# kit-cel/gr-gfdm

Hardware: AMD Instinct MI355X
Metric: GFDM blocks/s, K=64 M=9 mod+demod (MF), batch 4096 per GPU (higher is better)
Workload: dtype f32; 1 GPU; BASELINE configs[1]: K=64 subcarriers, M=9 timeslots, RRC alpha=0.2, overlap=2, MF receiver, step = modulate + demodulate; 4096 QPSK blocks per step per GPU, ring of 36 buffer sets, independent steps pipelined over 3 HIP streams; block_size=576, batch_per_gpu=4096, streams=3

## Files before the change

gr-gfdm_amd/csrc/gfdm_jit.hip:

```cpp
#include "gfdm_rowvariants.h"

#include <hip/hiprtc.h>

#include <fcntl.h>
#include <pthread.h>
#include <sys/stat.h>
#include <unistd.h>

#include <cstdio>
#include <cstdlib>
#include <cstring>
#include <atomic>
#include <condition_variable>
#include <deque>
#include <map>
#include <memory>
#include <mutex>
#include <thread>
#include <string>
#include <tuple>
#include <vector>

namespace gfdm {
namespace {

struct Header { const char* name; const char* text; };
const Header kHeaders[] = {
#include "gfdm_jit_sources.inc"
};
constexpr int kNumHeaders = sizeof(kHeaders) / sizeof(kHeaders[0]);
#define GFDM_JIT_STR_I(x) #x
#define GFDM_JIT_STR(x) GFDM_JIT_STR_I(x)
const char* const kOptions[] = { "--offload-arch=gfx950", "-O3", "-std=c++17", "-fno-slp-vectorize",
                                 "-DGFDM_PACKED_TWT=" GFDM_JIT_STR(GFDM_PACKED_TWT), "-DGFDM_PACKED_ROOTS=" GFDM_JIT_STR(GFDM_PACKED_ROOTS) };
constexpr int kNumOptions = sizeof(kOptions) / sizeof(kOptions[0]);

std::vector<std::string> part_kernels(int K, int M, int L, int part)
{
    char buf[160];
    std::vector<std::string> v;
    const rowvar::PartVariants t = rowvar::part_variants(K, M, part);
    for (int i = 0; i < t.n; ++i) {
        const rowvar::Variant& k = t.v[i];
        if (part == JIT_PART_MOD) snprintf(buf, sizeof buf, "gfdm::jit::k_row_modulate<%d, %d, %d, %d>", K, M, L, k.tx);
        else if (part == JIT_PART_EST) snprintf(buf, sizeof buf, "gfdm::jit::k_row_estimate<%d, %d>", K, M);
        else if (part == JIT_PART_RX_BURST) snprintf(buf, sizeof buf, "gfdm::jit::k_row_receive_burst<%d, %d, %d, %d, %d>", K, M, L, k.mode, k.ick);
        else snprintf(buf, sizeof buf, "gfdm::jit::k_row_receive<%d, %d, %d, %d, %d, %d>", K, M, L, k.mode, k.eq, k.ick);
        v.push_back(buf);
    }
    return v;
}

uint64_t fnv1a(uint64_t h, const void* data, size_t n)
{
    const unsigned char* p = static_cast<const unsigned char*>(data);
    for (size_t i = 0; i < n; ++i) { h ^= p[i]; h *= 1099511628211ull; }
    return h;
}

uint64_t source_hash()
{
    static const uint64_t h = [] {
        uint64_t x = 1469598103934665603ull;
        for (int i = 0; i < kNumHeaders; ++i) x = fnv1a(x, kHeaders[i].text, strlen(kHeaders[i].text));
        for (int i = 0; i < kNumOptions; ++i) x = fnv1a(x, kOptions[i], strlen(kOptions[i]));
        int major = 0, minor = 0;
        (void)hiprtcVersion(&major, &minor);
        x = fnv1a(x, &major, sizeof major);
        return fnv1a(x, &minor, sizeof minor);
    }();
    return h;
}

std::string cache_dir()
{
    std::string d;
    if (const char* e = getenv("GFDM_HIP_CACHE_DIR")) d = e;
    else if (const char* x = getenv("XDG_CACHE_HOME")) d = std::string(x) + "/gfdm_hip";
    else if (const char* h = getenv("HOME")) d = std::string(h) + "/.cache/gfdm_hip";
    if (d.empty()) return d;
    struct stat st;
    if (lstat(d.c_str(), &st) != 0)
        for (size_t i = 1; i <= d.size(); ++i)
            if (i == d.size() || d[i] == '/') (void)mkdir(d.substr(0, i).c_str(), i == d.size() ? 0700 : 0755);
    if (lstat(d.c_str(), &st) != 0 || !S_ISDIR(st.st_mode) || st.st_uid != getuid() || (st.st_mode & (S_IWGRP | S_IWOTH))) return std::string();
    return d;
}
// ... 365 lines not shown
```

gr-gfdm_amd/csrc/gfdm_rowgeom.h:

```cpp
#pragma once
#ifndef __HIPCC_RTC__
#include <stddef.h>
#endif

#ifndef GFDM_ROW_WG
#define GFDM_ROW_WG 256
#endif

namespace gfdm {
namespace rowgeom {

constexpr bool pow2(int K) { return K > 0 && (K & (K - 1)) == 0; }
constexpr int ldiv(int K, int lim)
{
    int r = 1;
    for (int d = 2; d <= lim && d <= K; ++d)
        if (K % d == 0) r = d;
    return r;
}
constexpr bool plan2(int K, int lim) { return K / ldiv(K, lim) <= lim; }
constexpr bool plan3(int K, int lim) { return ldiv(K, lim) > 1 && ldiv(K / ldiv(K, lim), lim) > 1 && plan2(K / ldiv(K, lim), lim); }
constexpr int plan_lim(int K) { return ((K <= 256 && plan2(K, 16)) || plan3(K, 16)) ? 16 : 32; }
constexpr bool mixed(int K)
{
    return !pow2(K) && K >= 3 && K <= 1024 && ((K <= 256 && plan2(K, 16)) || (!plan3(K, 16) && plan2(K, 32)));
}
constexpr int mixed_r1(int K) { return ldiv(K, plan_lim(K)); }
constexpr int mixed_r0(int K) { return K / mixed_r1(K); }
constexpr bool mixed3(int K)
{
    return !pow2(K) && !mixed(K) && K >= 3 && K <= 1024 && (plan3(K, 16) || plan3(K, 32));
}
constexpr int mixed3_r2(int K) { return ldiv(K, plan_lim(K)); }
constexpr int mixed3_r1(int K) { return ldiv(K / mixed3_r2(K), plan_lim(K)); }
constexpr int mixed3_r0(int K) { return K / mixed3_r2(K) / mixed3_r1(K); }
constexpr bool supported(int K) { return (pow2(K) && K >= 4 && K <= 1024) || mixed(K) || mixed3(K); }

constexpr int wg(int K) { return K >= 128 ? K : pow2(K) ? GFDM_ROW_WG : (GFDM_ROW_WG / K) * K; }
constexpr bool wave_local(int K) { return K <= 64 && 64 % K == 0; }
constexpr int bpw(int K) { return wg(K) / K; }
constexpr int tile_stride(int K, int M) { return K * M + (bpw(K) > 1 ? 16 : 0); }
constexpr size_t lds_bytes(int K, int M) { return (size_t)bpw(K) * (size_t)tile_stride(K, M) * 8 + 64; }
constexpr bool ic_mfma(int K, int M) { return pow2(K) && K >= 16 && M >= 4 && M <= 16; }
constexpr bool ic_mfma_preferred(int K, int M) { return ic_mfma(K, M) && K >= 128; }
constexpr size_t ic_mfma_pad_bytes(int K) { return wave_local(K) ? 0 : (size_t)(K / 4) * 8; }
constexpr size_t ic_mfma_edge_bytes(int K) { return wave_local(K) ? 0 : (size_t)2 * (K / 64) * 2 * 2 * 4 * 8 + ic_mfma_pad_bytes(K); }
constexpr int est_stride(int K) { return K + 10; }
constexpr size_t est_bytes(int K) { return (size_t)bpw(K) * (size_t)est_stride(K) * 8; }

#ifndef GFDM_PACKED_TWT
#define GFDM_PACKED_TWT 1
#endif
#ifndef GFDM_PACKED_ROOTS
#define GFDM_PACKED_ROOTS 0
#endif
constexpr int wide_r0(int K) { return K == 256 ? 16 : K == 128 ? 8 : mixed(K) ? mixed_r0(K) : mixed3(K) ? mixed3_r0(K) : (K == 512 || K == 1024) ? 8 : 1; }
constexpr int wide_r1(int K) { return (K == 256 || K == 128) ? 16 : mixed(K) ? mixed_r1(K) : mixed3(K) ? mixed3_r1(K) : (K == 512 || K == 1024) ? 8 : 1; }
constexpr bool wide3(int K) { return K == 512 || K == 1024 || mixed3(K); }
constexpr bool wide(int K) { return K == 256 || K == 128 || mixed(K) || wide3(K); }
constexpr int root_count(int K)
{
    if (wide(K)) return (wide_r0(K) - 1) + (wide3(K) ? wide_r1(K) - 1 : 0);
    if (K == 64) return 3;
    int n = 0;
    for (int len = K; len >= 4; len /= 4)
        if (len / 4 > 1) n += 3;
    return n;
}
constexpr int root_index(int K, int lane, int i)
{
    if (wide(K)) {
        const int R0 = wide_r0(K), R1 = wide_r1(K);
        if (i < R0 - 1) return (lane % (K / R0)) * (i + 1) % K;
        return ((lane % (K / R1)) / R0) * R0 * (i - (R0 - 1) + 1) % K;
    }
    int str = 1;
    for (int s = 0; s < i / 3; ++s) str *= 4;
    return ((lane % (K / 4)) / str) * (i % 3 + 1) * str % K;
}
constexpr bool packed_twt(int K, int M)
{
    return GFDM_PACKED_TWT != 0 && M >= 3 && !(K == 128 && (M == 15 || M == 21)) && !(K == 4 && M == 16);
}
constexpr bool packed_roots(int K, int M)
{
    return GFDM_PACKED_ROOTS != 0 && root_count(K) >= 2 && !(K == 128 && M == 15) && !(K == 96 && M == 25);
}
constexpr size_t packed_elems(int n, int K) { return ((size_t)n * (size_t)K + 1) & ~(size_t)1; }
constexpr size_t packed_roots_offset(int K, int M) { return packed_elems(M, K); }

}
}
```

gr-gfdm_amd/csrc/gfdm_rowlane_impl.h:

```cpp
#pragma once
#include "gfdm_dft.h"
#include "gfdm_plan.h"
#include "gfdm_tx.h"
#include "gfdm_est.h"
#include "gfdm_burstfetch.h"
#include "gfdm_rowgeom.h"

#ifndef __HIPCC_RTC__
#include <cstdlib>
#endif

#ifdef __HIPCC_RTC__
#define GFDM_ROWLANE_NS jit
#else
#define GFDM_ROWLANE_NS
#endif

#ifndef GFDM_ROW_WG
#define GFDM_ROW_WG 256
#endif

namespace gfdm {
namespace GFDM_ROWLANE_NS {

using namespace dft;

#ifdef GFDM_STAMPS
__device__ unsigned long long* g_stamp_buf = nullptr;
#define GFDM_STAMP(slot)                                                                                         \
    do {                                                                                                         \
        asm volatile("s_waitcnt vmcnt(0) lgkmcnt(0)" ::: "memory");                                              \
        if (g_stamp_buf && (threadIdx.x & 63) == 0)                                                               \
            g_stamp_buf[((size_t)blockIdx.x * (blockDim.x / 64) + (threadIdx.x >> 6)) * 8 + (slot)] = __builtin_amdgcn_s_memrealtime(); \
    } while (0)
#else
#define GFDM_STAMP(slot) do { } while (0)
#endif

template <int K> struct RowShape {
    static_assert(rowgeom::supported(K), "row-lane family: K a power of two 4 .. 1024, or K <= 1024 a product of two or three factors <= 32 (gfdm_rowgeom.h)");
    static constexpr bool MIXED3 = rowgeom::mixed3(K);
    static constexpr bool MIXED = rowgeom::mixed(K);
    static constexpr int R0 = MIXED ? rowgeom::mixed_r0(K) : 1, R1 = MIXED ? rowgeom::mixed_r1(K) : 1;
    static constexpr int log2K = (K == 4) ? 2 : (K == 8) ? 3 : (K == 16) ? 4 : (K == 32) ? 5 : (K == 64) ? 6 : (K == 128) ? 7 : (K == 256) ? 8 : (K == 512) ? 9 : (K == 1024) ? 10 : 0;
    static constexpr int NP4 = log2K / 2;
    static constexpr bool HAS2 = (log2K & 1) != 0;
    static constexpr int WG = rowgeom::wg(K);
    static constexpr int BPW = rowgeom::bpw(K);
    static constexpr int RG = K / 4;
    static constexpr bool RADIX16 = (K == 256);
    static constexpr bool RADIX8X16 = (K == 128);
    static constexpr bool WIDE3 = (K == 512 || K == 1024) || MIXED3;
    static constexpr bool WIDE = RADIX16 || RADIX8X16 || MIXED || WIDE3;
    static constexpr int WIDE_R0 = (RADIX16 ? 16 : RADIX8X16 ? 8 : MIXED ? R0 : MIXED3 ? rowgeom::mixed3_r0(K) : WIDE3 ? 8 : 1);
    static constexpr int WIDE_R1 = (RADIX16 || RADIX8X16) ? 16 : MIXED ? R1 : MIXED3 ? rowgeom::mixed3_r1(K) : WIDE3 ? 8 : 1;
    static constexpr int WIDE_R2 = MIXED3 ? rowgeom::mixed3_r2(K) : WIDE3 ? K / 64 : 1;
    static constexpr bool LDS_REDUCE = MIXED || MIXED3;
};

template <int K>
__device__ __forceinline__ int wrap_k(int x)
{
    if constexpr (rowgeom::pow2(K)) return x & (K - 1); else return x % K;
}

constexpr int pow4(int s) { return 1 << (2 * s); }

template <int K>
__device__ __forceinline__ void block_sync()
{
    if constexpr (rowgeom::wave_local(K)) {
        __builtin_amdgcn_fence(__ATOMIC_ACQ_REL, "wavefront");
        __builtin_amdgcn_wave_barrier();
    } else {
        __syncthreads();
    }
}

template <int K, int M> struct RowTile {
    static constexpr int N = K * M;
    static constexpr int TS = rowgeom::tile_stride(K, M);
};

template <int K, int M> constexpr size_t row_lds_bytes() { return rowgeom::lds_bytes(K, M); }

template <int K> struct EstTile {
    static constexpr int FS = rowgeom::est_stride(K);
    static constexpr size_t bytes = rowgeom::est_bytes(K);
};

template <int K> struct FftLayout {
    static __device__ __forceinline__ int slot(int row)
    {
        if constexpr (RowShape<K>::RADIX8X16) {
            const int a = (row >> 5) & 3, c = row & 7;
            return (row & ~7) | ((c + 2 * a) & 7);
        } else if constexpr (RowShape<K>::RADIX16) {
            return (row & ~15) | ((row + (row >> 4)) & 15);
        } else if constexpr (K >= 64 && rowgeom::pow2(K) && !RowShape<K>::WIDE3) {
            const int b = (row >> 4) & 3, c = (row >> 2) & 3, d = row & 3;
            return (row & ~63) | (16 * b + 4 * ((c + b) & 3) + ((d + b) & 3));
        } else {
            return row;
        }
    }
};

template <int K> struct FftTwiddles {
    cf w[RowShape<K>::WIDE ? 1 : RowShape<K>::NP4][3];
    cf w16[RowShape<K>::WIDE_R0 > 1 ? RowShape<K>::WIDE_R0 - 1 : 1];
    cf wmid[RowShape<K>::WIDE3 ? RowShape<K>::WIDE_R1 - 1 : 1];
};

template <int K, int N, class F>
__device__ __forceinline__ void load_lane_packed(const cf* __restrict__ tab, int q, F&& put)
{
    static_for<0, N / 2>([&](auto ji) {
        constexpr int j = decltype(ji)::value;
        const v4f_io w = *reinterpret_cast<const v4f_io*>(tab + 2 * (j * K + q));
        put(std::integral_constant<int, 2 * j>{}, mk(w.x, w.y));
        put(std::integral_constant<int, 2 * j + 1>{}, mk(w.z, w.w));
    });
    if constexpr (N % 2 != 0) put(std::integral_constant<int, N - 1>{}, tab[(N / 2) * 2 * K + q]);
}

template <int K, int M>
__device__ __forceinline__ void load_row_twiddles(cf (&tw)[M], const cf* __restrict__ twT, int q)
{
    if constexpr (rowgeom::packed_twt(K, M)) load_lane_packed<K, M - 1>(twT, q, [&](auto ii, cf w) { tw[decltype(ii)::value + 1] = w; });
    else static_for<1, M>([&](auto mi) { constexpr int m = decltype(mi)::value; tw[m] = twT[m * K + q]; });
}
// ... 293 lines not shown

#ifndef GFDM_WIDE_MOD_IN
#define GFDM_WIDE_MOD_IN 1
#endif
#ifndef GFDM_WIDE_RX_OUT
#define GFDM_WIDE_RX_OUT 0
#endif
#ifndef GFDM_WIDE_RX_IN
#define GFDM_WIDE_RX_IN 0
#endif
#ifndef GFDM_WIDE_MOD_OUT
#define GFDM_WIDE_MOD_OUT 0
#endif
constexpr bool kWideModIn = GFDM_WIDE_MOD_IN != 0, kWideRxOut = GFDM_WIDE_RX_OUT != 0, kWideRxIn = GFDM_WIDE_RX_IN != 0, kWideModOut = GFDM_WIDE_MOD_OUT != 0;

__device__ __forceinline__ float dpp_pair_swap(float x)
{
    return __builtin_bit_cast(float, __builtin_amdgcn_update_dpp(0, __builtin_bit_cast(int, x), 0xB1, 0xF, 0xF, true));
}
__device__ __forceinline__ cf dpp_pair_swap(cf x) { return mk(dpp_pair_swap(x.x), dpp_pair_swap(x.y)); }

template <int M>
__device__ __forceinline__ void wide_block_to_tile(cf* X, const cf* __restrict__ src, int l)
{
    v4f_io w[M / 2 > 0 ? M / 2 : 1];
    cf tail = mk(0.f, 0.f);
    static_for<0, M / 2>([&](auto ii) { constexpr int i = decltype(ii)::value; w[i] = ld_stream2(src + 2 * (l + 64 * i)); });
    if constexpr (M % 2) tail = ld_stream(src + 64 * (M - 1) + l);
    static_for<0, M / 2>([&](auto ii) { constexpr int i = decltype(ii)::value; reinterpret_cast<v4f_io*>(X)[l + 64 * i] = w[i]; });
    if constexpr (M % 2) X[64 * (M - 1) + l] = tail;
}
template <int M>
__device__ __forceinline__ void wide_tile_to_block(cf* __restrict__ dst, int64_t base, const cf* X, int l)
{
    static_for<0, M / 2>([&](auto ii) { constexpr int i = decltype(ii)::value; st_stream2(dst, base + 2 * (l + 64 * i), reinterpret_cast<const v4f_io*>(X)[l + 64 * i]); });
    if constexpr (M % 2) st_stream(dst, base + 64 * (M - 1) + l, X[64 * (M - 1) + l]);
}

template <int M>
__device__ __forceinline__ void wide_load_rows(cf (&v)[M], const cf* __restrict__ src, int l)
{
    const bool odd = (l & 1) != 0;
    const cf* p = src + 64 * (l & 1) + (l & ~1);
    v4f_io w[M / 2 > 0 ? M / 2 : 1];
    static_for<0, M / 2>([&](auto ii) { constexpr int i = decltype(ii)::value; w[i] = ld_stream2(p + 128 * i); });
    if constexpr (M % 2) v[M - 1] = ld_stream(src + 64 * (M - 1) + l);
    static_for<0, M / 2>([&](auto ii) {
        constexpr int i = decltype(ii)::value;
        const cf a = mk(w[i].x, w[i].y), b = mk(w[i].z, w[i].w);
        const cf got = dpp_pair_swap(odd ? a : b);
        v[2 * i] = odd ? got : a;
        v[2 * i + 1] = odd ? b : got;
    });
}
template <int M>
__device__ __forceinline__ void wide_store_rows(cf* __restrict__ dst, int64_t base, const cf (&v)[M], int l)
{
    const bool odd = (l & 1) != 0;
    const int64_t at = base + 64 * (l & 1) + (l & ~1);
    static_for<0, M / 2>([&](auto ii) {
        constexpr int i = decltype(ii)::value;
        const cf got = dpp_pair_swap(odd ? v[2 * i] : v[2 * i + 1]);
        const cf a = odd ? got : v[2 * i], b = odd ? v[2 * i + 1] : got;
        st_stream2(dst, at + 128 * i, v4f_io{ a.x, a.y, b.x, b.y });
    });
    if constexpr (M % 2) st_stream(dst, base + 64 * (M - 1) + l, v[M - 1]);
}

template <bool TREAL>
__device__ __forceinline__ cf tap_fma(cf t, cf x, cf c)
{
    if constexpr (TREAL) return mk(fmaf(t.x, x.x, c.x), fmaf(t.x, x.y, c.y)); else return cfma(t, x, c);
}

__device__ __forceinline__ cf decide_point(cf x, const IcParams& ic)
{
    if (ic.decision == 1) {
        const float s = 0.70710678118654752f;
        return mk(x.x > 0.f ? s : -s, x.y > 0.f ? s : -s);
    }
    int idx = 0;
    if (ic.decision == 2) {
        idx = (x.x > 0.f);
    } else {
        float best = __builtin_huge_valf();
        for (int i = 0; i < ic.npoints; ++i) {
            const cf pt = ic.points[i];
            const float dr = x.x - pt.x, di = x.y - pt.y, d = dr * dr + di * di;
            if (d < best) { best = d; idx = i; }
        }
    }
    return ic.points[idx];
}



#ifndef GFDM_IC_REG_TRANSPOSE
#define GFDM_IC_REG_TRANSPOSE 0
#endif
constexpr bool kIcRegTranspose = GFDM_IC_REG_TRANSPOSE != 0;

typedef _Float16 ic_h8 __attribute__((ext_vector_type(8)));
typedef float ic_f4 __attribute__((ext_vector_type(4)));

template <int K, int M> struct IcMfma {
    static constexpr int KW = K < 64 ? K : 64;
// ... 128 lines not shown
                    cur[g4][c] = __builtin_amdgcn_mfma_f32_16x16x32_f16(afrag, nb, c0[g4][c], 0, 0, 0);
                    cur[g4][c] = __builtin_amdgcn_mfma_f32_16x16x32_f16(afrag2, nb, cur[g4][c], 0, 0, 0);
                });
            });
        }
        static_for<0, 4>([&](auto gi) {
            constexpr int g4 = decltype(gi)::value;
            cf* row = reinterpret_cast<cf*>(blk0) + grp_block(g4) * TS + pa(wbase + G * cn + (g4 % G), 4 * cr);
            static_for<0, 4>([&](auto ii) {
                constexpr int i = decltype(ii)::value;
                if (12 + i < M || 4 * cr + i < M) row[i] = mk(cur[g4][0][i], cur[g4][1][i]);
            });
        });
        block_sync<K>();
    }
};

#ifndef GFDM_IC_WAVES_PER_SIMD
#define GFDM_IC_WAVES_PER_SIMD 2
#endif
template <int K, int M, int EQ> constexpr int ic_mfma_waves_per_simd()
{
    constexpr size_t lds = ((EQ == EQ_PREAMBLE || EQ == EQ_BURST) ? rowgeom::lds_bytes(K, M + 2) + rowgeom::est_bytes(K) : rowgeom::lds_bytes(K, M)) + rowgeom::ic_mfma_edge_bytes(K);
    constexpr size_t per_cu = (160 * 1024) / ((lds + 511) / 512 * 512) * (size_t)(rowgeom::wg(K) / 64);
    return per_cu >= 4 * (size_t)GFDM_IC_WAVES_PER_SIMD ? GFDM_IC_WAVES_PER_SIMD : 2;
}
#ifndef GFDM_VALU_IC_WAVES_PER_SIMD
#define GFDM_VALU_IC_WAVES_PER_SIMD 1
#endif
#define GFDM_ROW_RECEIVE_BOUNDS(EQ_) __launch_bounds__(RowShape<K>::WG, ((MODE == RX_IC && ICK == ICK_MFMA) ? ic_mfma_waves_per_simd<K, M, EQ_>() : (MODE == RX_IC && K <= 64) ? GFDM_VALU_IC_WAVES_PER_SIMD : 1))
template <int K, int M, int L, int MODE, int EQT, int ICK>
__global__ GFDM_ROW_RECEIVE_BOUNDS(EQT) void k_row_receive(DevicePlan p, IcParams ic, EstPlan est, const cf* __restrict__ twT,
                                                                cf* __restrict__ out, const cf* __restrict__ in,
                                                                const cf* __restrict__ f_eq, int64_t nblocks)
{
    const BurstIo bio{};
#include "gfdm_rowlane_receive_body.h"
}

template <int K, int M, int L, int MODE, int ICK>
__global__ GFDM_ROW_RECEIVE_BOUNDS(EQ_BURST) void k_row_receive_burst(DevicePlan p, IcParams ic, EstPlan est, const cf* __restrict__ twT,
                                                                cf* __restrict__ out, const cf* __restrict__ in,
                                                                const cf* __restrict__ f_eq, int64_t nblocks, BurstIo bio)
{
    constexpr int EQT = EQ_BURST;
#include "gfdm_rowlane_receive_body.h"
}
#undef GFDM_ROW_RECEIVE_BOUNDS

template <int K, int M, int L, int TXMODE>
__global__ __launch_bounds__(RowShape<K>::WG) void k_row_modulate(DevicePlan p, TxParams tx, const cf* __restrict__ twT,
                                                                 cf* __restrict__ out, const cf* __restrict__ in, int64_t nblocks)
{
    using S = RowShape<K>;
    using T = RowTile<K, M>;
    constexpr int N = K * M;
    constexpr int PART = (M * L / 2 < M) ? (M * L / 2) : M;
    extern __shared__ __attribute__((aligned(16))) unsigned char smem[];
    const int g = threadIdx.x / K, q = threadIdx.x - g * K;
    const int64_t blk = (int64_t)blockIdx.x * S::BPW + g;
    const bool valid = blk < nblocks;
    const int64_t base = (valid ? blk : 0) * N;
    cf* X = reinterpret_cast<cf*>(smem) + g * T::TS;

    FftTwiddles<K> twd;
    load_fft_twiddles<K, rowgeom::packed_roots(K, M)>(twd, q, p.wK);
    constexpr bool PRE_TW = (M <= 16), PRE_TAPS = (L * M <= 24);
    cf twv[M], tapv[PRE_TAPS ? L * M : 1];
    if constexpr (PRE_TW) load_row_twiddles<K, M>(twv, twT, q);
    if constexpr (PRE_TAPS) static_for<0, L * M>([&](auto ii) { constexpr int i = decltype(ii)::value; tapv[i] = p.taps[i]; });
    auto tap = [&](auto ii) { constexpr int i = decltype(ii)::value; if constexpr (PRE_TAPS) return tapv[i]; else return p.taps[i]; };
    constexpr bool WIDE_IN = (K == 64 && TXMODE == 0 && kWideModIn), WIDE_OUT = (K == 64 && TXMODE == 0 && kWideModOut);
    const bool treal = (K == 64) ? (p.taps_real & PLAN_TAPS_REAL) != 0 : p.taps_real != 0;
    const bool wide = (K == 64) && (p.taps_real & PLAN_WIDE_IO) != 0;
    (void)wide;
    cf v[M];
    if constexpr (TXMODE == 0) {
        bool copied = false;
        if constexpr (WIDE_IN) {
            if (wide) { wide_block_to_tile<M>(X, in + base, q); copied = true; }
        }
        if (!copied) static_for<0, M>([&](auto ii) { constexpr int i = decltype(ii)::value; X[q + K * i] = ld_stream(in + base + q + K * i); });
        block_sync<K>();
        static_for<0, M>([&](auto mi) { constexpr int m = decltype(mi)::value; v[m] = X[q * M + m]; });
    } else {
        const cf* sym = in + (valid ? blk : 0) * (int64_t)tx.nin;
        static_for<0, M>([&](auto mi) { constexpr int m = decltype(mi)::value; v[m] = tx_symbol(tx, sym, M, q, m); });
    }
    dft_inplace<M, false>(v);
    constexpr float invN = 1.0f / (float)N;
    if constexpr (!(K == 64 && L == 2)) {
        static_for<0, M>([&](auto mi) { constexpr int m = decltype(mi)::value; X[q * M + m] = v[m]; });
        block_sync<K>();
    }
    auto filter = [&](auto real_tag) {
        constexpr bool TREAL = decltype(real_tag)::value;
        if constexpr (K == 64 && L == 2) {
            static_for<0, M>([&](auto mi) {
                constexpr int m = decltype(mi)::value;
                const cf up = mk(dpp_wave_rol1(v[m].x), dpp_wave_rol1(v[m].y));
                cf acc = mk(0.f, 0.f);
                if constexpr (m < PART) {
                    acc = tap_fma<TREAL>(tap(std::integral_constant<int, M + m>{}), up, acc);
                    acc = tap_fma<TREAL>(tap(std::integral_constant<int, m>{}), v[m], acc);
                }
                v[m] = acc;
            });
        } else {
            static_for<0, M>([&](auto mi) { constexpr int m = decltype(mi)::value; v[m] = mk(0.f, 0.f); });
            static_for<0, L>([&](auto ii) {
                constexpr int i = decltype(ii)::value;
                const cf* rb = X + wrap_k<K>(q - i + L / 2 + K) * M;
                static_for<0, PART>([&](auto mi) {
                    constexpr int m = decltype(mi)::value;
                    v[m] = tap_fma<TREAL>(tap(std::integral_constant<int, ((i + L / 2) % L) * M + m>{}), rb[m], v[m]);
                });
            });
        }
    };
    if (treal) filter(std::true_type{}); else filter(std::false_type{});
    block_sync<K>();
    constexpr bool REGPASS = (K == 64) && kRegFirstPass;
    static_for<0, M>([&](auto mi) { constexpr int m = decltype(mi)::value; v[m] = scale(v[m], invN); });
    if constexpr (REGPASS) {
        wave_fft_first_pass<M, true>(X, q, twd, v);
    } else {
        cf* xa = X + FftLayout<K>::slot(q) * M;
        static_for<0, M>([&](auto mi) { constexpr int m = decltype(mi)::value; xa[m] = v[m]; });
        block_sync<K>();
    }
    lds_subcarrier_fft<K, M, true, REGPASS ? 1 : 0>(X, q, twd);
    v[0] = X[q * M];
    if constexpr (!PRE_TW && rowgeom::packed_twt(K, M)) load_row_twiddles<K, M>(twv, twT, q);
    static_for<1, M>([&](auto mi) {
        constexpr int m = decltype(mi)::value;
        cf w;
        if constexpr (PRE_TW || rowgeom::packed_twt(K, M)) w = twv[m]; else w = twT[m * K + q];
        v[m] = cmulc(X[q * M + m], w);
    });
    dft_inplace<M, true>(v);
    if (valid) {
        if constexpr (TXMODE == 2) {
            static_for<0, M>([&](auto pi) { constexpr int pp = decltype(pi)::value; tx_store_sample(tx, blk, N, K * pp + q, v[pp]); });
            tx_store_preamble(tx, blk, q, K);
        } else {
            bool stored = false;
            if constexpr (WIDE_OUT) {
                if (wide) { wide_store_rows<M>(out, base, v, q); stored = true; }
            }
            if (!stored) static_for<0, M>([&](auto pi) { constexpr int pp = decltype(pi)::value; st_stream(out, base + K * pp + q, v[pp]); });
        }
    }
}

template <int K, int M>
__global__ __launch_bounds__(RowShape<K>::WG) void k_row_estimate(EstPlan est, cf* __restrict__ out, const cf* __restrict__ in,
                                                                 int64_t nframes)
{
    using S = RowShape<K>;
    using T = RowTile<K, M>;
    constexpr int N = K * M;
    static_assert(N >= 3 * K, "the tile must hold the [K][2] preamble view plus the smoothed estimate");
    extern __shared__ __attribute__((aligned(16))) unsigned char smem[];
    const int g = threadIdx.x / K, q = threadIdx.x - g * K;
    const int64_t blk = (int64_t)blockIdx.x * S::BPW + g;
    const bool valid = blk < nframes;
    cf* X = reinterpret_cast<cf*>(smem) + g * T::TS;
    cf* inter = reinterpret_cast<cf*>(smem + row_lds_bytes<K, M>()) + g * EstTile<K>::FS;
    cf* F = X + 2 * K;

    const cf* pre = in + (valid ? blk : 0) * (int64_t)(2 * K);
    const cf p0 = ld_stream(pre + q), p1 = ld_stream(pre + K + q);
    const cf inv0 = est.inv0[q], inv1 = est.inv1[q];
    FftTwiddles<K> twd;
    load_fft_twiddles<K>(twd, q, est.wK);
    constexpr bool REGPASS = (K == 64) && kRegFirstPass;
    if constexpr (REGPASS) {
        const cf halves[2] = { p0, p1 };
        wave_fft_first_pass<2, false>(X, q, twd, halves);
    } else {
        cf* xa = X + FftLayout<K>::slot(q) * 2;
        xa[0] = p0;
        xa[1] = p1;
        block_sync<K>();
    }
    lds_subcarrier_fft<K, 2, false, REGPASS ? 1 : 0>(X, q, twd);
    const cf eq = cfma(X[2 * q], inv0, cmul(X[2 * q + 1], inv1));
    const int pos = est_active_pos(q, est), n_est = est.n_est;
    if (pos >= 0) {
        inter[4 + pos] = eq;
        if (pos == 0) { inter[0] = eq; inter[1] = eq; inter[2] = eq; inter[3] = eq; }
        if (pos == n_est - 1) { inter[n_est + 4] = eq; inter[n_est + 5] = eq; inter[n_est + 6] = eq; inter[n_est + 7] = eq; }
    }
    block_sync<K>();
    if (est.dc_free) {
        if (q == 0) {
            const cf lo = inter[4 + est.A / 2 - 1], hi = inter[4 + est.A / 2 + 1];
            inter[4 + est.A / 2] = mk(0.5f * (lo.x + hi.x), 0.5f * (lo.y + hi.y));
        }
        block_sync<K>();
    }
    if (q < n_est) {
        cf acc = mk(0.f, 0.f);
        static_for<0, 9>([&](auto ti) {
            constexpr int t = decltype(ti)::value;
            const cf x = inter[q + t];
            acc.x += x.x * est.gauss[t];
            acc.y += x.y * est.gauss[t];
        });
        F[q] = acc;
    }
    block_sync<K>();
    cf lo, hi;
    est_row_segment(F, 1, q, est, lo, hi);
    block_sync<K>();
    const cf dlt = mk(hi.x - lo.x, hi.y - lo.y);
    constexpr float step = 1.0f / (float)M;
    static_for<0, M>([&](auto mi) {
// ... 13 lines not shown
```

gr-gfdm_amd/csrc/gfdm_rowlane_receive_body.h:

```cpp
    using S = RowShape<K>;
    constexpr bool BURST = (EQT == EQ_BURST);
    constexpr int EQ = BURST ? (int)EQ_PREAMBLE : EQT;
    constexpr int MS = (EQ == EQ_PREAMBLE) ? M + 2 : M;
    using T = RowTile<K, MS>;
    constexpr int N = K * M;
    constexpr bool ICSYM = (ICK == ICK_REALSYM);
    constexpr bool ICMX = (MODE == RX_IC && ICK == ICK_MFMA);
    static_assert(!ICMX || rowgeom::ic_mfma(K, M), "IcMfma: K a power of two >= 16, 4 <= M <= 16");
    extern __shared__ __attribute__((aligned(16))) unsigned char smem[];
    const int g = threadIdx.x / K, q = threadIdx.x - g * K;
    const int64_t blk = (int64_t)blockIdx.x * S::BPW + g;
    const bool valid = blk < nblocks;
    const int64_t base = (valid ? blk : 0) * N;
    const int64_t in_base = (valid ? blk : 0) * (int64_t)(ic.io.in_stride ? ic.io.in_stride : N) + ic.io.in_offset;
    cf* X = reinterpret_cast<cf*>(smem) + g * T::TS;

    GFDM_STAMP(0);
    bool live = valid;
    int64_t cap_base = 0, cap_len = 0;
    int cap_rotate = 0;
    double cap_phi = 0.0;
    (void)live; (void)cap_base; (void)cap_len; (void)cap_rotate; (void)cap_phi;
    if constexpr (BURST) {
        if (bio.count) {
            const int64_t cnt = *bio.count;
            live = blk < cnt;
        }
        live = live && valid;
        if (live) {
            cap_base = bio.off[blk] - bio.backoff;
            cap_len = bio.cap_len;
            if (bio.rot) burst_phase_step(bio.rot[blk], cap_rotate, cap_phi);
        }
    }
    cf v[M];
    constexpr bool WIDE_IN = (K == 64 && !BURST && kWideRxIn), WIDE_OUT = (K == 64 && !BURST && !ICMX && kWideRxOut);
    const bool wide = (K == 64) && (p.taps_real & PLAN_WIDE_IO) != 0;
    (void)wide;
    if constexpr (!BURST) {
        bool loaded = false;
        if constexpr (WIDE_IN) {
            if (wide) { wide_load_rows<M>(v, in + in_base, q); loaded = true; }
        }
        if (!loaded) static_for<0, M>([&](auto pi) { constexpr int pp = decltype(pi)::value; v[pp] = ld_stream(in + in_base + K * pp + q); });
    }
    FftTwiddles<K> twd;
    load_fft_twiddles<K, rowgeom::packed_roots(K, M)>(twd, q, p.wK);
    constexpr bool PRE_TAPS = (L * M <= 24);
    cf tapv[PRE_TAPS ? L * M : 1], icgv[(PRE_TAPS && MODE == RX_IC) ? M : 1];
    if constexpr (PRE_TAPS) {
        static_for<0, L * M>([&](auto ii) { constexpr int i = decltype(ii)::value; tapv[i] = p.taps[i]; });
        if constexpr (MODE == RX_IC) static_for<0, M>([&](auto ii) { constexpr int i = decltype(ii)::value; icgv[i] = p.icg[i]; });
    }
    auto tap = [&](auto ii) { constexpr int i = decltype(ii)::value; if constexpr (PRE_TAPS) return tapv[i]; else return p.taps[i]; };
    const bool treal = (K == 64) ? (p.taps_real & PLAN_TAPS_REAL) != 0 : p.taps_real != 0;
    auto icg = [&](auto ii) { constexpr int i = decltype(ii)::value; if constexpr (PRE_TAPS && MODE == RX_IC) return icgv[i]; else return p.icg[i]; };
    const int wgt = (MODE == RX_IC && !ICMX) ? ic.active[q] : 0;
    typename IcMfma<ICMX ? K : 16, ICMX ? M : 4>::Pre icpre;
    if constexpr (ICMX) IcMfma<K, M>::preload(icpre, p, ic);
    const int rank_q = (MODE != RX_FD && ic.io.demap) ? ic.io.rank[q] : -1;
    const int io_demap = ic.io.demap, io_nout = ic.io.nout, io_per_timeslot = ic.io.per_timeslot, io_A = ic.io.A;
    const int ic_iter = ic.ic_iter, ic_decision = ic.decision, ic_pc = ic.do_phase_compensation;
    GFDM_STAMP(1);
    cf pre0, pre1, inv0, inv1;
    if constexpr (BURST) {
        const int n0 = ic.io.in_offset + q, np = bio.pre + q;
        static_for<0, M>([&](auto pi) { constexpr int pp = decltype(pi)::value; v[pp] = burst_fetch(bio.cap, bio.fmt, cap_len, cap_base, n0 + K * pp, 1.f, cap_rotate, cap_phi); });
        pre0 = burst_fetch(bio.cap, bio.fmt, cap_len, cap_base, np, 1.f, cap_rotate, cap_phi);
        pre1 = burst_fetch(bio.cap, bio.fmt, cap_len, cap_base, np + K, 1.f, cap_rotate, cap_phi);
        inv0 = est.inv0[q];
        inv1 = est.inv1[q];
    } else if constexpr (EQ == EQ_PREAMBLE) {
        const cf* pre = f_eq + (valid ? blk : 0) * (int64_t)(est.pre_stride ? est.pre_stride : 2 * K);
        pre0 = ld_stream(pre + q);
        pre1 = ld_stream(pre + K + q);
        inv0 = est.inv0[q];
        inv1 = est.inv1[q];
    }
    cf tw[M];
    load_row_twiddles<K, M>(tw, twT, q);
    dft_inplace<M, false>(v);
    constexpr bool REGPASS = (K == 64) && kRegFirstPass;
    if constexpr (REGPASS) {
        cf rowv[MS];
        rowv[0] = v[0];
        static_for<1, M>([&](auto mi) { constexpr int m = decltype(mi)::value; rowv[m] = cmul(v[m], tw[m]); });
        if constexpr (EQ == EQ_PREAMBLE) { rowv[M] = pre0; rowv[M + 1] = pre1; }
        wave_fft_first_pass<MS, false>(X, q, twd, rowv);
    } else {
        cf* xa = X + FftLayout<K>::slot(q) * MS;
        xa[0] = v[0];
        static_for<1, M>([&](auto mi) { constexpr int m = decltype(mi)::value; xa[m] = cmul(v[m], tw[m]); });
        if constexpr (EQ == EQ_PREAMBLE) { xa[M] = pre0; xa[M + 1] = pre1; }
        block_sync<K>();
    }
    constexpr bool ROWREG = (K == 64 && L == 2 && EQ == EQ_PREAMBLE && !(ICMX && kIcRegTranspose));
    cf xrow[ROWREG ? M : 1];
    cf heq[EQ == EQ_VECTOR ? M : 1];
    if constexpr (EQ == EQ_VECTOR) {
        __builtin_amdgcn_sched_barrier(0);
        static_for<0, M>([&](auto ii) { constexpr int i = decltype(ii)::value; heq[i] = ld_stream(f_eq + base + q + K * i); });
    }

    lds_subcarrier_fft<K, MS, false, REGPASS ? 1 : 0>(X, q, twd);

    GFDM_STAMP(2);
    if constexpr (EQ == EQ_VECTOR) {
        static_for<0, M>([&](auto ii) {
            constexpr int i = decltype(ii)::value;
            const cf a = X[q + K * i], b = heq[i];
            const float inv = __builtin_amdgcn_rcpf(b.x * b.x + b.y * b.y);
            X[q + K * i] = mk((a.x * b.x + a.y * b.y) * inv, (a.y * b.x - a.x * b.y) * inv);
        });
        block_sync<K>();
    } else if constexpr (EQ == EQ_PREAMBLE) {
        cf* inter = reinterpret_cast<cf*>(smem + row_lds_bytes<K, MS>()) + g * EstTile<K>::FS;
        cf* F = X + M;
        const cf eq = cfma(X[q * MS + M], inv0, cmul(X[q * MS + M + 1], inv1));
        const int pos = est_active_pos(q, est), n_est = est.n_est;
        if (pos >= 0) {
            inter[4 + pos] = eq;
            if (pos == 0) { inter[0] = eq; inter[1] = eq; inter[2] = eq; inter[3] = eq; }
            if (pos == n_est - 1) { inter[n_est + 4] = eq; inter[n_est + 5] = eq; inter[n_est + 6] = eq; inter[n_est + 7] = eq; }
        }
        block_sync<K>();
        if (est.dc_free) {
            if (q == 0) {
                const cf lo = inter[4 + est.A / 2 - 1], hi = inter[4 + est.A / 2 + 1];
                inter[4 + est.A / 2] = mk(0.5f * (lo.x + hi.x), 0.5f * (lo.y + hi.y));
            }
            block_sync<K>();
        }
        if (q < n_est) {
// ... 142 lines not shown
            } else {
                static_for<0, M>([&](auto pi) {
                    constexpr int pp = decltype(pi)::value;
                    cf acc = d0[pp];
                    static_for<0, M>([&](auto ri) {
                        constexpr int r = decltype(ri)::value;
                        const cf g = icg(std::integral_constant<int, r>{}), x = nb[(pp - r + M) % M];
                        acc = mk(fmaf(-g.x, x.x, fmaf(g.y, x.y, acc.x)), fmaf(-g.x, x.y, fmaf(-g.y, x.x, acc.y)));
                    });
                    d[pp] = acc;
                });
            }
            if constexpr (K != 64) block_sync<K>();
        }
    }

    GFDM_STAMP(4);
    if (MODE != RX_FD && io_demap) {
        const int a = rank_q;
        if constexpr (ICMX) static_for<0, M>([&](auto mi) { constexpr int m = decltype(mi)::value; d[m] = X[IcMfma<ICMX ? K : 16, ICMX ? M : 4>::pa(q, m)]; });
        if (valid && a >= 0) {
            cf* o = out + blk * (int64_t)io_nout;
            static_for<0, M>([&](auto mi) {
                constexpr int m = decltype(mi)::value;
                const int idx = io_per_timeslot ? (m * io_A + a) : (a * M + m);
                if constexpr (BURST) { if (idx < io_nout) st_stream(o, idx, live ? d[m] : mk(0.f, 0.f)); }
                else if (idx < io_nout) st_stream(o, idx, d[m]);
            });
        }
    } else {
        if constexpr (!ICMX) {
            static_for<0, M>([&](auto mi) { constexpr int m = decltype(mi)::value; X[q * M + m] = (MODE == RX_FD) ? s[m] : d[m]; });
            block_sync<K>();
        }
        if constexpr (BURST) {
            if (valid) static_for<0, M>([&](auto ii) {
                constexpr int i = decltype(ii)::value;
                cf r;
                if constexpr (ICMX) r = X[IcMfma<ICMX ? K : 16, ICMX ? M : 4>::pa_linear(q + K * i)]; else r = X[q + K * i];
                st_stream(out, base + q + K * i, live ? r : mk(0.f, 0.f));
            });
        } else if (valid) {
            if constexpr (ICMX) static_for<0, M>([&](auto ii) { constexpr int i = decltype(ii)::value; st_stream(out, base + q + K * i, X[IcMfma<ICMX ? K : 16, ICMX ? M : 4>::pa_linear(q + K * i)]); });
            else {
                bool stored = false;
                if constexpr (WIDE_OUT) {
                    if (wide) { wide_tile_to_block<M>(out, base, X, q); stored = true; }
                }
                if (!stored) static_for<0, M>([&](auto ii) { constexpr int i = decltype(ii)::value; st_stream(out, base + q + K * i, X[q + K * i]); });
            }
        }
    }
    GFDM_STAMP(5);
```

gr-gfdm_amd/csrc/gfdm_rowvariants.h:

```cpp
#pragma once
#include "gfdm_plan.h"
#include "gfdm_tx.h"
#include "gfdm_rowgeom.h"

#include <atomic>
#include <cstdint>
#include <cstdlib>

namespace gfdm {
namespace rowvar {

struct Variant { int part, mode, eq, ick, tx; };

constexpr int kMaxVariants = 6;
struct PartVariants {
    int part = 0, n = 0;
    Variant v[kMaxVariants] = {};
    constexpr void add(int mode, int eq, int ick, int tx = 0) { v[n++] = Variant{ part, mode, eq, ick, tx }; }
};

constexpr PartVariants part_variants(int K, int M, int part)
{
    PartVariants t{ part };
    const bool mx = rowgeom::ic_mfma(K, M);
// ... 37 lines not shown
    return Choice{ want, -1 };
}

inline Choice select_receive(const DevicePlan& p, const IcParams& ic, const EstPlan* est, int mode, const cf* f_eq)
{
    const bool rounds = (mode == RX_IC && ic.ic_iter > 0);
    const int ick = !rounds ? ICK_GENERAL : (ic_mfma_applies(p, ic) && rowgeom::ic_mfma(p.K, p.M)) ? ICK_MFMA : p.ic_real_sym ? ICK_REALSYM : ICK_GENERAL;
    const bool gather = burst_io(est) != nullptr;
    return find(p.K, p.M, Variant{ gather ? JIT_PART_RX_BURST : est ? JIT_PART_RX_PREAMBLE : rounds ? JIT_PART_RX_IC : JIT_PART_RX,
                                   mode == RX_FD ? RX_FD : rounds ? RX_IC : RX_DEMOD, gather ? EQ_BURST : est ? EQ_PREAMBLE : f_eq ? EQ_VECTOR : EQ_NONE, ick, 0 });
}

inline Choice select_modulate(const DevicePlan& p, const TxParams& tx)
{
    return find(p.K, p.M, Variant{ JIT_PART_MOD, 0, EQ_NONE, ICK_GENERAL, (tx.mapped && tx.framed) ? 2 : tx.mapped ? 1 : 0 });
}

inline std::atomic<int>& wide_access()
{
    static std::atomic<int> on{ [] { const char* e = getenv("GFDM_HIP_WIDE_ACCESS"); return (e && e[0] == '0' && !e[1]) ? 0 : 1; }() };
    return on;
}

inline bool aligned16(const void* a) { return (reinterpret_cast<uintptr_t>(a) & 15u) == 0; }

inline int plan_flags_modulate(const DevicePlan& p, const TxParams& tx, const cf* out, const cf* in)
{
    const bool wide = p.K == 64 && !tx.mapped && !tx.framed && aligned16(out) && aligned16(in) && wide_access().load(std::memory_order_relaxed) != 0;
    return p.taps_real | (wide ? (int)PLAN_WIDE_IO : 0);
}

inline int plan_flags_receive(const DevicePlan& p, const IcParams& ic, const EstPlan* est, const cf* out, const cf* in, const cf* f_eq)
{
    const bool wide = p.K == 64 && !burst_io(est) && ic.io.in_stride == 0 && ic.io.in_offset == 0 && aligned16(out) && aligned16(in) && aligned16(f_eq) &&
                      wide_access().load(std::memory_order_relaxed) != 0;
    return p.taps_real | (wide ? (int)PLAN_WIDE_IO : 0);
}

inline const cf* plan_roots(const DevicePlan& p, const cf* twT)
{
    return rowgeom::packed_roots(p.K, p.M) ? twT + rowgeom::packed_roots_offset(p.K, p.M) : p.wK;
}

inline Choice select_estimate(const EstPlan& e) { return find(e.K, e.M, Variant{ JIT_PART_EST, 0, EQ_NONE, ICK_GENERAL, 0 }); }

struct Geometry { unsigned grid, block; size_t lds; };

constexpr Geometry geometry(int K, int M, const Variant& v, int64_t nblocks)
{
    const bool pre = (v.eq == EQ_PREAMBLE || v.eq == EQ_BURST);
    size_t lds = rowgeom::lds_bytes(K, pre ? M + 2 : M);
    if (pre || v.part == JIT_PART_EST) lds += rowgeom::est_bytes(K);
    if (v.ick == ICK_MFMA) lds += rowgeom::ic_mfma_edge_bytes(K);
    return Geometry{ (unsigned)((nblocks + rowgeom::bpw(K) - 1) / rowgeom::bpw(K)), (unsigned)rowgeom::wg(K), lds };
}

inline hipError_t allow_lds(const void* f, size_t lds)
{
    return lds > 64 * 1024 ? hipFuncSetAttribute(f, hipFuncAttributeMaxDynamicSharedMemorySize, (int)lds) : hipSuccess;
}

}
}
```

Baseline: 307.3 million blocks/s.

## Add configurable multi-round persistent workgroups and separate wave-local workgroup size

Adds compile-time knobs GFDM_ROW_WG_LOCAL and GFDM_ROW_ROUNDS. With more than one round, each workgroup of the modulate and receive kernels loops over several block groups, so per-thread FFT and row twiddles and filter taps are loaded once and reused across blocks. The grid shrinks to match. Defaults (256, 1 round) keep the old geometry, apart from 16-element tile padding now also applied to wave-local K=64 tiles. The round loop is compiled out at default settings.

```diff
diff --git a/gr-gfdm_amd/csrc/gfdm_jit.hip b/gr-gfdm_amd/csrc/gfdm_jit.hip
--- a/gr-gfdm_amd/csrc/gfdm_jit.hip
+++ b/gr-gfdm_amd/csrc/gfdm_jit.hip
@@ -32,7 +32,9 @@
 #define GFDM_JIT_STR_I(x) #x
 #define GFDM_JIT_STR(x) GFDM_JIT_STR_I(x)
 const char* const kOptions[] = { "--offload-arch=gfx950", "-O3", "-std=c++17", "-fno-slp-vectorize",
-                                 "-DGFDM_PACKED_TWT=" GFDM_JIT_STR(GFDM_PACKED_TWT), "-DGFDM_PACKED_ROOTS=" GFDM_JIT_STR(GFDM_PACKED_ROOTS) };
+                                 "-DGFDM_PACKED_TWT=" GFDM_JIT_STR(GFDM_PACKED_TWT), "-DGFDM_PACKED_ROOTS=" GFDM_JIT_STR(GFDM_PACKED_ROOTS),
+                                 "-DGFDM_ROW_WG=" GFDM_JIT_STR(GFDM_ROW_WG), "-DGFDM_ROW_WG_LOCAL=" GFDM_JIT_STR(GFDM_ROW_WG_LOCAL),
+                                 "-DGFDM_ROW_ROUNDS=" GFDM_JIT_STR(GFDM_ROW_ROUNDS) };
 constexpr int kNumOptions = sizeof(kOptions) / sizeof(kOptions[0]);
 
 std::vector<std::string> part_kernels(int K, int M, int L, int part)
diff --git a/gr-gfdm_amd/csrc/gfdm_rowgeom.h b/gr-gfdm_amd/csrc/gfdm_rowgeom.h
--- a/gr-gfdm_amd/csrc/gfdm_rowgeom.h
+++ b/gr-gfdm_amd/csrc/gfdm_rowgeom.h
@@ -6,6 +6,14 @@
 #ifndef GFDM_ROW_WG
 #define GFDM_ROW_WG 256
 #endif
+#ifndef GFDM_ROW_WG_LOCAL
+#define GFDM_ROW_WG_LOCAL 256
+#endif
+#ifndef GFDM_ROW_ROUNDS
+#define GFDM_ROW_ROUNDS 1
+#endif
+static_assert(GFDM_ROW_WG_LOCAL == 64 || GFDM_ROW_WG_LOCAL == 128 || GFDM_ROW_WG_LOCAL == 256, "GFDM_ROW_WG_LOCAL: 64, 128 or 256");
+static_assert(GFDM_ROW_ROUNDS == 1 || GFDM_ROW_ROUNDS == 2 || GFDM_ROW_ROUNDS == 4, "GFDM_ROW_ROUNDS: 1, 2 or 4");
 
 namespace gfdm {
 namespace rowgeom {
@@ -36,10 +44,21 @@
 constexpr int mixed3_r0(int K) { return K / mixed3_r2(K) / mixed3_r1(K); }
 constexpr bool supported(int K) { return (pow2(K) && K >= 4 && K <= 1024) || mixed(K) || mixed3(K); }
 
-constexpr int wg(int K) { return K >= 128 ? K : pow2(K) ? GFDM_ROW_WG : (GFDM_ROW_WG / K) * K; }
 constexpr bool wave_local(int K) { return K <= 64 && 64 % K == 0; }
+constexpr int wg(int K) { return K >= 128 ? K : wave_local(K) ? GFDM_ROW_WG_LOCAL : (GFDM_ROW_WG / K) * K; }
 constexpr int bpw(int K) { return wg(K) / K; }
-constexpr int tile_stride(int K, int M) { return K * M + (bpw(K) > 1 ? 16 : 0); }
+enum { PART_RX = 0, PART_RX_IC = 1, PART_RX_PREAMBLE = 2, PART_MOD = 3, PART_EST = 4, PART_RX_BURST = 5 };
+constexpr int rounds(int K, int part)
+{
+    return (wave_local(K) && (part == PART_RX || part == PART_RX_IC || part == PART_MOD)) ? GFDM_ROW_ROUNDS : 1;
+}
+constexpr int blocks_per_wg(int K, int part) { return bpw(K) * rounds(K, part); }
+constexpr long long block_index(int K, int part, long long workgroup, int round, int g)
+{
+    return (workgroup * rounds(K, part) + round) * bpw(K) + g;
+}
+constexpr long long grid_size(int K, int part, long long nblocks) { return (nblocks + blocks_per_wg(K, part) - 1) / blocks_per_wg(K, part); }
+constexpr int tile_stride(int K, int M) { return K * M + ((bpw(K) > 1 || wave_local(K)) ? 16 : 0); }
 constexpr size_t lds_bytes(int K, int M) { return (size_t)bpw(K) * (size_t)tile_stride(K, M) * 8 + 64; }
 constexpr bool ic_mfma(int K, int M) { return pow2(K) && K >= 16 && M >= 4 && M <= 16; }
 constexpr bool ic_mfma_preferred(int K, int M) { return ic_mfma(K, M) && K >= 128; }
diff --git a/gr-gfdm_amd/csrc/gfdm_rowlane_impl.h b/gr-gfdm_amd/csrc/gfdm_rowlane_impl.h
--- a/gr-gfdm_amd/csrc/gfdm_rowlane_impl.h
+++ b/gr-gfdm_amd/csrc/gfdm_rowlane_impl.h
@@ -14,10 +14,6 @@
 #define GFDM_ROWLANE_NS jit
 #else
 #define GFDM_ROWLANE_NS
-#endif
-
-#ifndef GFDM_ROW_WG
-#define GFDM_ROW_WG 256
 #endif
 
 namespace gfdm {
@@ -77,6 +73,19 @@
     }
 }
 
+template <int K>
+__device__ __forceinline__ int wave_first_group()
+{
+    return __builtin_amdgcn_readfirstlane((int)threadIdx.x) / K;
+}
+
+template <int ROUNDS>
+__device__ __forceinline__ int per_round(int x)
+{
+    if constexpr (ROUNDS > 1) asm volatile("" : "+v"(x));
+    return x;
+}
+
 template <int K, int M> struct RowTile {
     static constexpr int N = K * M;
     static constexpr int TS = rowgeom::tile_stride(K, M);
@@ -476,6 +485,15 @@
         v[2 * i] = odd ? got : a;
         v[2 * i + 1] = odd ? b : got;
     });
+}
+template <int K, int M, bool WIDE_IN>
+__device__ __forceinline__ void load_block_samples(cf (&v)[M], const cf* src, int q, bool wide)
+{
+    bool loaded = false;
+    if constexpr (WIDE_IN) {
+        if (wide) { wide_load_rows<M>(v, src, q); loaded = true; }
+    }
+    if (!loaded) static_for<0, M>([&](auto pi) { constexpr int pp = decltype(pi)::value; v[pp] = ld_stream(src + K * pp + q); });
 }
 template <int M>
 __device__ __forceinline__ void wide_store_rows(cf* __restrict__ dst, int64_t base, const cf (&v)[M], int l)
@@ -710,15 +728,16 @@
 __global__ __launch_bounds__(RowShape<K>::WG) void k_row_modulate(DevicePlan p, TxParams tx, const cf* __restrict__ twT,
                                                                  cf* __restrict__ out, const cf* __restrict__ in, int64_t nblocks)
 {
-    using S = RowShape<K>;
     using T = RowTile<K, M>;
     constexpr int N = K * M;
     constexpr int PART = (M * L / 2 < M) ? (M * L / 2) : M;
+    constexpr int ROUNDS = rowgeom::rounds(K, rowgeom::PART_MOD);
     extern __shared__ __attribute__((aligned(16))) unsigned char smem[];
-    const int g = threadIdx.x / K, q = threadIdx.x - g * K;
-    const int64_t blk = (int64_t)blockIdx.x * S::BPW + g;
-    const bool valid = blk < nblocks;
-    const int64_t base = (valid ? blk : 0) * N;
+    const int g = threadIdx.x / K;
+    int q = threadIdx.x - g * K;
+    int64_t blk = rowgeom::block_index(K, rowgeom::PART_MOD, blockIdx.x, 0, g);
+    bool valid = blk < nblocks;
+    int64_t base = (valid ? blk : 0) * N;
     cf* X = reinterpret_cast<cf*>(smem) + g * T::TS;
 
     FftTwiddles<K> twd;
@@ -733,6 +752,19 @@
     const bool wide = (K == 64) && (p.taps_real & PLAN_WIDE_IO) != 0;
     (void)wide;
     cf v[M];
+#if GFDM_ROW_ROUNDS > 1
+    int round = 0;
+    do {
+    if constexpr (ROUNDS > 1) {
+        if (round > 0) {
+            if (rowgeom::block_index(K, rowgeom::PART_MOD, blockIdx.x, round, wave_first_group<K>()) >= nblocks) break;
+            blk = rowgeom::block_index(K, rowgeom::PART_MOD, blockIdx.x, round, g);
+            valid = blk < nblocks;
+            base = (valid ? blk : 0) * N;
+            q = per_round<ROUNDS>(q);
+        }
+    }
+#endif
     if constexpr (TXMODE == 0) {
         bool copied = false;
         if constexpr (WIDE_IN) {
@@ -809,19 +841,22 @@
             if (!stored) static_for<0, M>([&](auto pi) { constexpr int pp = decltype(pi)::value; st_stream(out, base + K * pp + q, v[pp]); });
         }
     }
+#if GFDM_ROW_ROUNDS > 1
+    if constexpr (ROUNDS > 1) block_sync<K>();
+    } while (ROUNDS > 1 && ++round < ROUNDS);
+#endif
 }
 
 template <int K, int M>
 __global__ __launch_bounds__(RowShape<K>::WG) void k_row_estimate(EstPlan est, cf* __restrict__ out, const cf* __restrict__ in,
                                                                  int64_t nframes)
 {
-    using S = RowShape<K>;
     using T = RowTile<K, M>;
     constexpr int N = K * M;
     static_assert(N >= 3 * K, "the tile must hold the [K][2] preamble view plus the smoothed estimate");
     extern __shared__ __attribute__((aligned(16))) unsigned char smem[];
     const int g = threadIdx.x / K, q = threadIdx.x - g * K;
-    const int64_t blk = (int64_t)blockIdx.x * S::BPW + g;
+    const int64_t blk = rowgeom::block_index(K, rowgeom::PART_EST, blockIdx.x, 0, g);
     const bool valid = blk < nframes;
     cf* X = reinterpret_cast<cf*>(smem) + g * T::TS;
     cf* inter = reinterpret_cast<cf*>(smem + row_lds_bytes<K, M>()) + g * EstTile<K>::FS;
diff --git a/gr-gfdm_amd/csrc/gfdm_rowlane_receive_body.h b/gr-gfdm_amd/csrc/gfdm_rowlane_receive_body.h
--- a/gr-gfdm_amd/csrc/gfdm_rowlane_receive_body.h
+++ b/gr-gfdm_amd/csrc/gfdm_rowlane_receive_body.h
@@ -8,11 +8,14 @@
     constexpr bool ICMX = (MODE == RX_IC && ICK == ICK_MFMA);
     static_assert(!ICMX || rowgeom::ic_mfma(K, M), "IcMfma: K a power of two >= 16, 4 <= M <= 16");
     extern __shared__ __attribute__((aligned(16))) unsigned char smem[];
-    const int g = threadIdx.x / K, q = threadIdx.x - g * K;
-    const int64_t blk = (int64_t)blockIdx.x * S::BPW + g;
-    const bool valid = blk < nblocks;
-    const int64_t base = (valid ? blk : 0) * N;
-    const int64_t in_base = (valid ? blk : 0) * (int64_t)(ic.io.in_stride ? ic.io.in_stride : N) + ic.io.in_offset;
+    constexpr int RPART = BURST ? rowgeom::PART_RX_BURST : (EQ == EQ_PREAMBLE) ? rowgeom::PART_RX_PREAMBLE : (MODE == RX_IC) ? rowgeom::PART_RX_IC : rowgeom::PART_RX;
+    constexpr int ROUNDS = rowgeom::rounds(K, RPART);
+    const int g = threadIdx.x / K;
+    int q = threadIdx.x - g * K;
+    int64_t blk = rowgeom::block_index(K, RPART, blockIdx.x, 0, g);
+    bool valid = blk < nblocks;
+    int64_t base = (valid ? blk : 0) * N;
+    int64_t in_base = (valid ? blk : 0) * (int64_t)(ic.io.in_stride ? ic.io.in_stride : N) + ic.io.in_offset;
     cf* X = reinterpret_cast<cf*>(smem) + g * T::TS;
 
     GFDM_STAMP(0);
@@ -37,13 +40,7 @@
     constexpr bool WIDE_IN = (K == 64 && !BURST && kWideRxIn), WIDE_OUT = (K == 64 && !BURST && !ICMX && kWideRxOut);
     const bool wide = (K == 64) && (p.taps_real & PLAN_WIDE_IO) != 0;
     (void)wide;
-    if constexpr (!BURST) {
-        bool loaded = false;
-        if constexpr (WIDE_IN) {
-            if (wide) { wide_load_rows<M>(v, in + in_base, q); loaded = true; }
-        }
-        if (!loaded) static_for<0, M>([&](auto pi) { constexpr int pp = decltype(pi)::value; v[pp] = ld_stream(in + in_base + K * pp + q); });
-    }
+    if constexpr (!BURST) load_block_samples<K, M, WIDE_IN>(v, in + in_base, q, wide);
     FftTwiddles<K> twd;
     load_fft_twiddles<K, rowgeom::packed_roots(K, M)>(twd, q, p.wK);
     constexpr bool PRE_TAPS = (L * M <= 24);
@@ -79,6 +76,21 @@
     }
     cf tw[M];
     load_row_twiddles<K, M>(tw, twT, q);
+#if GFDM_ROW_ROUNDS > 1
+    int round = 0;
+    do {
+    if constexpr (ROUNDS > 1) {
+        if (round > 0) {
+            if (rowgeom::block_index(K, RPART, blockIdx.x, round, wave_first_group<K>()) >= nblocks) break;
+            blk = rowgeom::block_index(K, RPART, blockIdx.x, round, g);
+            valid = blk < nblocks;
+            base = (valid ? blk : 0) * N;
+            in_base = (valid ? blk : 0) * (int64_t)(ic.io.in_stride ? ic.io.in_stride : N) + ic.io.in_offset;
+            q = per_round<ROUNDS>(q);
+            if constexpr (!BURST) load_block_samples<K, M, WIDE_IN>(v, in + in_base, q, wide);
+        }
+    }
+#endif
     dft_inplace<M, false>(v);
     constexpr bool REGPASS = (K == 64) && kRegFirstPass;
     if constexpr (REGPASS) {
@@ -327,3 +339,7 @@
         }
     }
     GFDM_STAMP(5);
+#if GFDM_ROW_ROUNDS > 1
+    if constexpr (ROUNDS > 1) block_sync<K>();
+    } while (ROUNDS > 1 && ++round < ROUNDS);
+#endif
diff --git a/gr-gfdm_amd/csrc/gfdm_rowvariants.h b/gr-gfdm_amd/csrc/gfdm_rowvariants.h
--- a/gr-gfdm_amd/csrc/gfdm_rowvariants.h
+++ b/gr-gfdm_amd/csrc/gfdm_rowvariants.h
@@ -113,8 +113,11 @@
     size_t lds = rowgeom::lds_bytes(K, pre ? M + 2 : M);
     if (pre || v.part == JIT_PART_EST) lds += rowgeom::est_bytes(K);
     if (v.ick == ICK_MFMA) lds += rowgeom::ic_mfma_edge_bytes(K);
-    return Geometry{ (unsigned)((nblocks + rowgeom::bpw(K) - 1) / rowgeom::bpw(K)), (unsigned)rowgeom::wg(K), lds };
+    return Geometry{ (unsigned)rowgeom::grid_size(K, v.part, nblocks), (unsigned)rowgeom::wg(K), lds };
 }
+static_assert(JIT_PART_RX == rowgeom::PART_RX && JIT_PART_RX_IC == rowgeom::PART_RX_IC && JIT_PART_RX_PREAMBLE == rowgeom::PART_RX_PREAMBLE &&
+              JIT_PART_MOD == rowgeom::PART_MOD && JIT_PART_EST == rowgeom::PART_EST && JIT_PART_RX_BURST == rowgeom::PART_RX_BURST,
+              "rowgeom::rounds() names the parts by the values of JIT_PART_*");
 
 inline hipError_t allow_lds(const void* f, size_t lds)
 {
```

New measurement: 306.5 million blocks/s, median of 2. About the same (-0.3%).
